# hustvl/LSFA

Hardware: AMD Instinct MI355X
Metric: frames/sec/GPU at 1000x600 key_interval=10 (whole-job frames/s) (higher is better)
Workload: dtype f32

## Files before the change

### lsfa_amd/csrc/conv_ring_kernel.h

```cpp
#pragma once
#include "conv_split_kernel.h"

namespace lsfa {
namespace convsplit {

constexpr int kFlush = 12;

#ifndef LSFA_RING_A_AUX
#define LSFA_RING_A_AUX 0
#endif
#ifndef LSFA_RING_B_AUX
#define LSFA_RING_B_AUX 0
#endif

#ifdef LSFA_LAB_HALF_A
constexpr int kRingIssueA = 2;
#else
constexpr int kRingIssueA = 4;
#endif

template <int NT, int PC, int ST, int WV = 4> struct Ring {
  static constexpr int kColTile = 128 * PC;
  static constexpr int kStageA = WV * 256;
  static constexpr int kStageBn = NT * kColTile;
  static constexpr int kStageN = kStageA + kStageBn;
  static constexpr int kDmaB = (NT * kColTile) / (WV * 64);
  static constexpr int kDma = kRingIssueA + kDmaB;
  static constexpr int kLdsBytes = ST * kStageN * 16;
  static constexpr int kWgPerCu = (2 * kLdsBytes <= 160 * 1024) ? 2 : 1;
  static_assert((NT * kColTile) % (WV * 64) == 0, "NT * PC must be a multiple of WV / 2");
  static_assert(kLdsBytes <= 160 * 1024, "ring does not fit the CU's LDS");
  static_assert((ST - 1) * kDma <= 63, "vmcnt is a 6-bit counter");
};

__device__ __forceinline__ float4 affine_relu4(const float4& v, const float4& sc, const float4& sh) {
  return make_float4(fmaxf(v.x * sc.x + sh.x, 0.f), fmaxf(v.y * sc.y + sh.y, 0.f), fmaxf(v.z * sc.z + sh.z, 0.f), fmaxf(v.w * sc.w + sh.w, 0.f));
}
__device__ __forceinline__ void affine_chunk(const float* T, int gch, int lane, float4& c0, float4& c1, float4& c2, float4& c3) {
  const float4* sc = reinterpret_cast<const float4*>(T + gch * kChunk + 16 * (lane >> 5));
  const float4* sh = reinterpret_cast<const float4*>(T + kAffineMaxCin + gch * kChunk + 16 * (lane >> 5));
  c0 = affine_relu4(c0, sc[0], sh[0]);
  c1 = affine_relu4(c1, sc[1], sh[1]);
  c2 = affine_relu4(c2, sc[2], sh[2]);
  c3 = affine_relu4(c3, sc[3], sh[3]);
}

template <int NT, int PC, int ST, int WV, int S>
__device__ __forceinline__ void ring_issue_a(uint4 (*R)[(Ring<NT, PC, ST, WV>::kStageN)], const float* __restrict__ x, const Geom& g, const Walk& wk, bool live) {
  const int dy = wk.ty * g.dil, dx = wk.tx * g.dil;
  const int doff = (dy * g.W + dx) * g.lda + wk.kc * kChunk;
  const int dy_b = live ? dy : (1 << 26);
  uint4* a_dst = &R[S][g.wave * 256];
#pragma unroll
  for (int i = 0; i < kRingIssueA; ++i) {
    const bool ok = (unsigned)(g.iy0[i] + dy_b) < (unsigned)g.H && (unsigned)(g.ix0[i] + dx) < (unsigned)g.W;
    const float* src = ok ? x + (g.off0[i] + doff) : g_zero_block;
    __builtin_amdgcn_global_load_lds(reinterpret_cast<const uint4*>(src), a_dst + i * 64, 16, 0, LSFA_RING_A_AUX);
  }
}

template <int NT, int PC, int ST, int WV, int S, int I0, int I1>
__device__ __forceinline__ void ring_issue_b(uint4 (*R)[(Ring<NT, PC, ST, WV>::kStageN)], const uint4* __restrict__ wblock, const Geom& g, int gch) {
  typedef Ring<NT, PC, ST, WV> RG;
  const uint4* wsrc = wblock + (size_t)gch * g.wstride + g.wave * (RG::kDmaB * 64) + g.lane;
  uint4* b_dst = &R[S][RG::kStageA + g.wave * (RG::kDmaB * 64)];
#pragma unroll
  for (int i = I0; i < I1; ++i) __builtin_amdgcn_global_load_lds(wsrc + i * 64, b_dst + i * 64, 16, 0, LSFA_RING_B_AUX);
}

template <int NT, int PC, int ST, int WV, int S, bool PIPE>
__device__ __forceinline__ void ring_issue_chunk(uint4 (*R)[(Ring<NT, PC, ST, WV>::kStageN)], const float* __restrict__ x, const uint4* __restrict__ wblock,
                                                 const Geom& g, Walk& wk, bool live) {
  ring_issue_a<NT, PC, ST, WV, S>(R, x, g, wk, PIPE ? live : true);
  ring_issue_b<NT, PC, ST, WV, S, 0, Ring<NT, PC, ST, WV>::kDmaB>(R, wblock, g, PIPE ? wk.bprev : wk.bidx);
  wk.next(g.kh, g.kw, g.chunks_per_tap, g.k_order);
}

template <int NT, int PC, int ST, int WV, int S, bool PIPE, bool GUARD>
__device__ __forceinline__ void ring_prologue(uint4 (*R)[(Ring<NT, PC, ST, WV>::kStageN)], const float* __restrict__ x, const uint4* __restrict__ wblock,
                                              const Geom& g, Walk& wk, int n) {
  if (!GUARD || S < n) ring_issue_chunk<NT, PC, ST, WV, S, PIPE>(R, x, wblock, g, wk, S + 1 < n);
}

template <int ST, int kDma>
__device__ __forceinline__ void wait_chunks_ahead(int ahead) {
  if (ST >= 4 && ahead >= 2) wait_vmcnt<(ST >= 4 ? 2 : 0) * kDma>();
  else if (ST >= 3 && ahead == 1) wait_vmcnt<(ST >= 3 ? 1 : 0) * kDma>();
  else wait_vmcnt<0>();
}

struct Cut { PiecesN s0, s1; };

template <int PC, bool AF>
__device__ __forceinline__ Cut cut_rows(const uint4& r0, const uint4& r1, const uint4& r2, const uint4& r3, float a_scale, const float* T, int gch, int lane) {
  float4 c0 = as_f4(r0), c1 = as_f4(r1), c2 = as_f4(r2), c3 = as_f4(r3);
  if (AF) affine_chunk(T, gch, lane, c0, c1, c2, c3);
  Cut n;
  n.s0 = cut8<PC>(c0, c1, AF ? 1.f : a_scale);
  n.s1 = cut8<PC>(c2, c3, AF ? 1.f : a_scale);
  return n;
}

template <int PC, bool AF> struct CutCost { static constexpr int kValu = (PC == 2 ? 64 : PC == 3 ? 96 : 16) + (AF ? 48 : 0); };

template <int NT, int PC, bool AF, int DMA = 0, int WV = 4> __device__ __forceinline__ void pin_interleave() {
  if (PC == 3 && NT == 4) return;
  constexpr int kMfma = NT * 2 * (PC == 3 ? 6 : PC == 2 ? 3 : 1);
  constexpr int kPer = (CutCost<PC, AF>::kValu + (DMA ? 24 : 0) + kMfma - 1) / kMfma + 1;
  __builtin_amdgcn_sched_group_barrier(0x100, ((PC == 3 || WV == 8) ? PC + 2 : 2 * PC + 4) + (AF ? 8 : 0), 0);
#pragma unroll
  for (int i = 0; i < kMfma; ++i) {
    __builtin_amdgcn_sched_group_barrier(0x008, 1, 0);
    __builtin_amdgcn_sched_group_barrier(0x100, 1, 0);
    if (i >= 1 && i <= DMA) __builtin_amdgcn_sched_group_barrier(0x010, 1, 0);
    __builtin_amdgcn_sched_group_barrier(0x002, kPer, 0);
  }
}

template <int NT, int PC, int ST, int WV, int S, bool AF, int DMA = 0>
__device__ __forceinline__ Cut ring_mma_cut(const uint4 (*R)[(Ring<NT, PC, ST, WV>::kStageN)], const Geom& g, const Cut& p, f32x16 (&acc)[NT], float a_scale,
                                            int gch_next, const float* T) {
  const uint4* B = &R[S][Ring<NT, PC, ST, WV>::kStageA + g.lane];
  const uint4* A = &R[S][g.wave * 256];
  uint4 bf[NT * 2][PC];
#pragma unroll
  for (int q = 0; q < PC; ++q) bf[0][q] = B[q * 64];
  const uint4 r0 = A[g.frag[0]], r1 = A[g.frag[1]];
#pragma unroll
  for (int t = 1; t < NT; ++t)
#pragma unroll
    for (int q = 0; q < PC; ++q) bf[t * 2][q] = B[((t * 2) * PC + q) * 64];
  const uint4 r2 = A[g.frag[2]], r3 = A[g.frag[3]];
#pragma unroll
  for (int t = 0; t < NT; ++t)
#pragma unroll
    for (int q = 0; q < PC; ++q) bf[t * 2 + 1][q] = B[((t * 2 + 1) * PC + q) * 64];
  const Cut n = cut_rows<PC, AF>(r0, r1, r2, r3, a_scale, T, min(gch_next, g.chunks_per_tap - 1), g.lane);
#pragma unroll
  for (int t = 0; t < NT; ++t) acc[t] = mma_pc<PC>(p.s0, bf[t * 2][0], bf[t * 2][PC > 1 ? 1 : 0], bf[t * 2][PC > 2 ? 2 : 0], acc[t]);
#pragma unroll
  for (int t = 0; t < NT; ++t) acc[t] = mma_pc<PC>(p.s1, bf[t * 2 + 1][0], bf[t * 2 + 1][PC > 1 ? 1 : 0], bf[t * 2 + 1][PC > 2 ? 2 : 0], acc[t]);
  pin_interleave<NT, PC, AF, DMA, WV>();
  return n;
}

template <int NT, int PC, int ST, int WV, int S, bool AF>
__device__ __forceinline__ Cut ring_cut(const uint4 (*R)[(Ring<NT, PC, ST, WV>::kStageN)], const Geom& g, float a_scale, int gch, const float* T) {
  const uint4* A = &R[S][g.wave * 256];
  const uint4 r0 = A[g.frag[0]], r1 = A[g.frag[1]], r2 = A[g.frag[2]], r3 = A[g.frag[3]];
  return cut_rows<PC, AF>(r0, r1, r2, r3, a_scale, T, min(gch, g.chunks_per_tap - 1), g.lane);
}

template <int NT, int PC, int ST, int WV, int S, bool AF>
__device__ __forceinline__ void ring_step_uniform(uint4 (*R)[(Ring<NT, PC, ST, WV>::kStageN)], const float* __restrict__ x, const uint4* __restrict__ wblock,
                                                  const Geom& g, Walk& wk, int v, int n, f32x16 (&acc)[NT], Cut& p, float a_scale, const float* T) {
  typedef Ring<NT, PC, ST, WV> RG;
  constexpr int SN = (S + ST - 1) % ST;
  wait_vmcnt<(ST - 2) * RG::kDma>();
  asm volatile("s_waitcnt lgkmcnt(0)" ::: "memory");
  __builtin_amdgcn_s_barrier();
  const Walk cur = wk;
  wk.next(g.kh, g.kw, g.chunks_per_tap, g.k_order);
  ring_issue_a<NT, PC, ST, WV, SN>(R, x, g, cur, v + ST < n);
  ring_issue_b<NT, PC, ST, WV, SN, 0, RG::kDmaB>(R, wblock, g, cur.bprev);
  p = ring_mma_cut<NT, PC, ST, WV, S, AF, RG::kDma>(R, g, p, acc, a_scale, g.chunk0 + v + 1, T);
}

template <int NT, int PC, int ST, int WV, int S, bool PIPE>
__device__ __forceinline__ void ring_load_step(uint4 (*R)[(Ring<NT, PC, ST, WV>::kStageN)], const float* __restrict__ x, const uint4* __restrict__ wblock,
                                               const Geom& g, Walk& wk, int v, int n) {
  typedef Ring<NT, PC, ST, WV> RG;
  constexpr int SN = (S + ST - 1) % ST;
  wait_chunks_ahead<ST, RG::kDma>(min(n - 1 - v, ST - 2));
  __builtin_amdgcn_s_barrier();
  if (v + ST - 1 < n) ring_issue_chunk<NT, PC, ST, WV, SN, PIPE>(R, x, wblock, g, wk, v + ST < n);
}

template <int NT, int PC, int ST, int WV, int S, bool AF>
__device__ __forceinline__ void ring_consume_step(uint4 (*R)[(Ring<NT, PC, ST, WV>::kStageN)], const Geom& g, f32x16 (&acc)[NT], Cut& p, float a_scale, int v,
                                                  const float* T) {
  asm volatile("s_waitcnt lgkmcnt(0)" ::: "memory");
  __builtin_amdgcn_s_barrier();
  p = ring_mma_cut<NT, PC, ST, WV, S, AF>(R, g, p, acc, a_scale, g.chunk0 + v + 1, T);
}

template <int NT, int PC, int ST, int WV>
__device__ __forceinline__ void ring_wait_first(int n) {
  typedef Ring<NT, PC, ST, WV> RG;
  const int behind = min(n, ST - 1);
  if (ST >= 4 && behind >= 3) wait_vmcnt<(ST >= 4 ? 3 : 0) * RG::kDma>();
  else if (ST >= 3 && behind == 2) wait_vmcnt<(ST >= 3 ? 2 : 0) * RG::kDma>();
  else if (behind == 1) wait_vmcnt<RG::kDma>();
  else wait_vmcnt<0>();
}

template <int NT, int PC, int ST, int S, bool AF, bool COPIES>
__device__ __forceinline__ void ring_step_r4(uint4 (*R)[(Ring<NT, PC, ST, 4>::kStageN)], const float* __restrict__ x, const uint4* __restrict__ wblock,
                                          const Geom& g, Walk& wk, int c, int n, f32x16 (&acc)[NT], float a_scale, const float* T) {
  typedef Ring<NT, PC, ST, 4> RG;
  constexpr int kDmaB = RG::kDmaB;
  constexpr int SN = (S + ST - 1) % ST;
  if (COPIES) wait_chunks_ahead<ST, RG::kDma>(min(n - 1 - c, ST - 2));
  asm volatile("s_waitcnt lgkmcnt(0)" ::: "memory");
  __builtin_amdgcn_s_barrier();
  const bool more = COPIES && c + ST - 1 < n;
  const int gch_next = wk.bidx;
  if (more) ring_issue_a<NT, PC, ST, 4, SN>(R, x, g, wk, true);
  const uint4* A = &R[S][g.wave * 256];
  const uint4* B = &R[S][Ring<NT, PC, ST, 4>::kStageA + g.lane];
  const uint4 r0 = A[g.frag[0]], r1 = A[g.frag[1]], r2 = A[g.frag[2]], r3 = A[g.frag[3]];
  float4 c0 = as_f4(r0), c1 = as_f4(r1), c2 = as_f4(r2), c3 = as_f4(r3);
  if (AF) affine_chunk(T, g.chunk0 + c, g.lane, c0, c1, c2, c3);
  const PiecesN s0 = cut8<PC>(c0, c1, AF ? 1.f : a_scale), s1 = cut8<PC>(c2, c3, AF ? 1.f : a_scale);
#pragma unroll
  for (int t = 0; t < NT; ++t) {
    acc[t] = mma_pc<PC>(s0, B + ((t * 2 + 0) * PC) * 64, acc[t]);
    acc[t] = mma_pc<PC>(s1, B + ((t * 2 + 1) * PC) * 64, acc[t]);
    if (more) {
      constexpr int kPer = (kDmaB + NT - 1) / NT;
      constexpr int kE0 = (kPer < kDmaB) ? kPer : kDmaB;
      constexpr int kE1 = (2 * kPer < kDmaB) ? 2 * kPer : kDmaB;
      constexpr int kE2 = (3 * kPer < kDmaB) ? 3 * kPer : kDmaB;
      if (t == 0) ring_issue_b<NT, PC, ST, 4, SN, 0, kE0>(R, wblock, g, gch_next);
      if (NT > 1 && t == 1) ring_issue_b<NT, PC, ST, 4, SN, kE0, (NT > 2 ? kE1 : kDmaB)>(R, wblock, g, gch_next);
      if (NT > 2 && t == 2) ring_issue_b<NT, PC, ST, 4, SN, kE1, (NT > 3 ? kE2 : kDmaB)>(R, wblock, g, gch_next);
      if (NT > 3 && t == 3) ring_issue_b<NT, PC, ST, 4, SN, kE2, kDmaB>(R, wblock, g, gch_next);
    }
  }
  if (more) wk.next(g.kh, g.kw, g.chunks_per_tap, g.k_order);
}

template <int NT, int PC, int ST, bool SP = false, bool AF = false, int WV = 4>
static __global__ __launch_bounds__((SP || WV == 8 ? 2 : 1) * kThreads,
    WV == 8 ? 2 : (((AF ? 2 * (Ring<NT, PC, ST, WV>::kLdsBytes + 16384) <= 160 * 1024 : Ring<NT, PC, ST, WV>::kWgPerCu == 2) && !(SP && NT == 4)) ? 2 : 1) * (SP ? 2 : 1))
void conv_ring_kernel(Args a, int nx, int ny, int nz) {
  typedef Ring<NT, PC, ST, WV> RG;
  __shared__ __attribute__((aligned(16))) uint4 R[ST][RG::kStageN];
  __shared__ __attribute__((aligned(16))) float T[AF ? 2 * kAffineMaxCin : 4];
  Tile tile = xcd_tile(blockIdx.x, nx, ny, nz, a.tile_order, a.inv_nx, a.inv_ny);
  if (tile.x < 0) return;
  if (a.nphase > 1) { const int slices = nz / a.nphase, phase = tile.z / slices; tile.z -= phase * slices; apply_phase(a, phase, slices); }
  const int tid = threadIdx.x;
  const int P = a.N * a.Ho * a.Wo;
  static_assert(!(SP && WV != 4), "loader / consumer waves exist for 128-pixel tiles only");
  constexpr int kPix = 32 * WV;
  constexpr bool kUniform = !SP && (WV == 8 || NT == 4);
  constexpr bool kPipelined = (SP && NT == 4) || kUniform;
  if (tile.x * kPix >= P) return;
  const int taps = a.kh * a.kw;
  Geom g;
  g.lane = tid & 63;
  const int wave8 = __builtin_amdgcn_readfirstlane(tid >> 6);
  const bool loader = SP && wave8 >= 4;
  g.wave = WV == 8 ? wave8 : (wave8 & 3);
  float a_scale = 1.f;
  float out_scale[NT];
#pragma unroll
  for (int t = 0; t < NT; ++t) out_scale[t] = 1.f;
  ScaleRegs sr;
  if (PC == 2 && !loader) scale_loads_issue<NT>(a, tile.y * (32 * NT), g.lane, sr);
#ifdef LSFA_LAB_EARLY_SCALES
  constexpr bool kScalesEarly = true;
#else
  constexpr bool kScalesEarly = false;
#endif
#define LSFA_SCALES_READY(N_)                                                                                                   \
  if (!kScalesEarly || (N_) < 0) {                                                                                              \
    if (PC == 2) { scale_loads_wait<((N_) < 0 ? 0 : (N_))>(sr); a_scale = scale_finish<NT>(a, sr, g.lane, out_scale); }         \
    if (AF) {                                                                                                                   \
      for (int k = tid; k < a.Cin; k += 64 * WV) { T[k] = a.in_scale[k] * a_scale; T[kAffineMaxCin + k] = a.in_shift[k] * a_scale; } \
    }                                                                                                                           \
  }
  if (kScalesEarly && !loader) LSFA_SCALES_READY(-1)
  g.H = a.H; g.W = a.W; g.Cin = a.Cin; g.lda = a.lda; g.kh = a.kh; g.kw = a.kw; g.stride = a.stride; g.dil = a.dil;
  g.k_order = taps > 1 ? a.k_order : 0;
  g.chunks_per_tap = a.Cin / kChunk;
  const int chunk_total = taps * g.chunks_per_tap;
  g.chunk0 = tile.z * a.chunks_per_slice;
  const int nchunks = min(a.chunks_per_slice, chunk_total - g.chunk0);
  const int col_tiles = a.Cout / 32;
  g.wstride = (size_t)col_tiles * RG::kColTile;
  const uint4* wblock = a.wfrag + (size_t)(NT * tile.y) * RG::kColTile;
  const int m0 = tile.x * kPix + g.wave * kWavePix;
  if (!SP || loader) {
#pragma unroll
  for (int i = 0; i < 4; ++i) {
    const int pix = m0 + 8 * i + (g.lane >> 3);
    const int piece = LSFA_DMA_SRC_PIECE(i, g.lane);
    g.iy0[i] = g.ix0[i] = -(1 << 24);
    g.off0[i] = 0;
    if (pix < P) {
      const int pn = fdiv(pix, a.Ho * a.Wo, a.inv_howo), r = pix - pn * a.Ho * a.Wo, py = fdiv(r, a.Wo, a.inv_wo), px = r - py * a.Wo;
      g.iy0[i] = py * a.stride - a.pad_h;
      g.ix0[i] = px * a.stride - a.pad_w;
      g.off0[i] = ((pn * a.H + g.iy0[i]) * a.W + g.ix0[i]) * a.lda + 4 * piece;
    }
  }
  }
  LSFA_FRAG_SLOTS(g.lane, g.frag)
  f32x16 acc[NT];
#pragma unroll
  for (int t = 0; t < NT; ++t)
#pragma unroll
    for (int i = 0; i < 16; ++i) acc[t][i] = 0.f;

  Walk wk;
  wk.start(g.chunk0, a.kh, a.kw, g.chunks_per_tap, g.k_order);
  f32x16 sum[NT];
#pragma unroll
  for (int t = 0; t < NT; ++t)
#pragma unroll
    for (int i = 0; i < 16; ++i) sum[t][i] = 0.f;
  if constexpr (!kPipelined) {
    if (SP) {
      if (loader) {
        ring_prologue<NT, PC, ST, 4, 0, false, true>(R, a.x, wblock, g, wk, nchunks);
        if (ST > 2) ring_prologue<NT, PC, ST, 4, (ST > 2 ? 1 : 0), false, true>(R, a.x, wblock, g, wk, nchunks);
        if (ST > 3) ring_prologue<NT, PC, ST, 4, (ST > 3 ? 2 : 0), false, true>(R, a.x, wblock, g, wk, nchunks);
        for (int c = 0; c < nchunks; c += ST) {
          ring_load_step<NT, PC, ST, 4, 0, false>(R, a.x, wblock, g, wk, c, nchunks);
          if (c + 1 < nchunks) ring_load_step<NT, PC, ST, 4, 1, false>(R, a.x, wblock, g, wk, c + 1, nchunks);
          if (ST > 2 && c + 2 < nchunks) ring_load_step<NT, PC, ST, 4, (ST > 2 ? 2 : 0), false>(R, a.x, wblock, g, wk, c + 2, nchunks);
          if (ST > 3 && c + 3 < nchunks) ring_load_step<NT, PC, ST, 4, (ST > 3 ? 3 : 0), false>(R, a.x, wblock, g, wk, c + 3, nchunks);
        }
        return;
      }
      LSFA_SCALES_READY(0)
      int since = 0;
      for (int c = 0; c < nchunks; c += ST) {
        ring_step_r4<NT, PC, ST, 0, AF, false>(R, a.x, wblock, g, wk, c, nchunks, acc, a_scale, T);
        if (c + 1 < nchunks) ring_step_r4<NT, PC, ST, 1, AF, false>(R, a.x, wblock, g, wk, c + 1, nchunks, acc, a_scale, T);
        if (ST > 2 && c + 2 < nchunks) ring_step_r4<NT, PC, ST, (ST > 2 ? 2 : 0), AF, false>(R, a.x, wblock, g, wk, c + 2, nchunks, acc, a_scale, T);
        if (ST > 3 && c + 3 < nchunks) ring_step_r4<NT, PC, ST, (ST > 3 ? 3 : 0), AF, false>(R, a.x, wblock, g, wk, c + 3, nchunks, acc, a_scale, T);
        since += ST;
        if (since >= kFlush) {
          since = 0;
  #pragma unroll
          for (int t = 0; t < NT; ++t)
  #pragma unroll
            for (int i = 0; i < 16; ++i) { sum[t][i] = sum[t][i] + acc[t][i]; acc[t][i] = 0.f; }
        }
      }
    } else {
      ring_prologue<NT, PC, ST, 4, 0, false, true>(R, a.x, wblock, g, wk, nchunks);
      if (ST > 2) ring_prologue<NT, PC, ST, 4, (ST > 2 ? 1 : 0), false, true>(R, a.x, wblock, g, wk, nchunks);
      if (ST > 3) ring_prologue<NT, PC, ST, 4, (ST > 3 ? 2 : 0), false, true>(R, a.x, wblock, g, wk, nchunks);
      LSFA_SCALES_READY(0)
      int since = 0;
      for (int c = 0; c < nchunks; c += ST) {
        ring_step_r4<NT, PC, ST, 0, AF, true>(R, a.x, wblock, g, wk, c, nchunks, acc, a_scale, T);
        if (c + 1 < nchunks) ring_step_r4<NT, PC, ST, 1, AF, true>(R, a.x, wblock, g, wk, c + 1, nchunks, acc, a_scale, T);
        if (ST > 2 && c + 2 < nchunks) ring_step_r4<NT, PC, ST, (ST > 2 ? 2 : 0), AF, true>(R, a.x, wblock, g, wk, c + 2, nchunks, acc, a_scale, T);
        if (ST > 3 && c + 3 < nchunks) ring_step_r4<NT, PC, ST, (ST > 3 ? 3 : 0), AF, true>(R, a.x, wblock, g, wk, c + 3, nchunks, acc, a_scale, T);
        since += ST;
        if (since >= kFlush) {
          since = 0;
  #pragma unroll
          for (int t = 0; t < NT; ++t)
  #pragma unroll
            for (int i = 0; i < 16; ++i) { sum[t][i] = sum[t][i] + acc[t][i]; acc[t][i] = 0.f; }
        }
      }
    }
  } else {
  if (SP && loader) {
    ring_issue_a<NT, PC, ST, WV, ST - 1>(R, a.x, g, wk, true);
    wk.next(g.kh, g.kw, g.chunks_per_tap, g.k_order);
    ring_prologue<NT, PC, ST, WV, 0, true, true>(R, a.x, wblock, g, wk, nchunks);
    if (ST > 2) ring_prologue<NT, PC, ST, WV, (ST > 2 ? 1 : 0), true, true>(R, a.x, wblock, g, wk, nchunks);
    if (ST > 3) ring_prologue<NT, PC, ST, WV, (ST > 3 ? 2 : 0), true, true>(R, a.x, wblock, g, wk, nchunks);
    ring_wait_first<NT, PC, ST, WV>(nchunks);
    __builtin_amdgcn_s_barrier();
    for (int c = 0; c < nchunks; c += ST) {
      ring_load_step<NT, PC, ST, WV, 0, true>(R, a.x, wblock, g, wk, c, nchunks);
      if (c + 1 < nchunks) ring_load_step<NT, PC, ST, WV, 1, true>(R, a.x, wblock, g, wk, c + 1, nchunks);
      if (ST > 2 && c + 2 < nchunks) ring_load_step<NT, PC, ST, WV, (ST > 2 ? 2 : 0), true>(R, a.x, wblock, g, wk, c + 2, nchunks);
      if (ST > 3 && c + 3 < nchunks) ring_load_step<NT, PC, ST, WV, (ST > 3 ? 3 : 0), true>(R, a.x, wblock, g, wk, c + 3, nchunks);
    }
    return;
  }
  if (kUniform) {
    ring_issue_a<NT, PC, ST, WV, ST - 1>(R, a.x, g, wk, true);
    wk.next(g.kh, g.kw, g.chunks_per_tap, g.k_order);
    ring_prologue<NT, PC, ST, WV, 0, true, false>(R, a.x, wblock, g, wk, nchunks);
    if (ST > 2) ring_prologue<NT, PC, ST, WV, (ST > 2 ? 1 : 0), true, false>(R, a.x, wblock, g, wk, nchunks);
    if (ST > 3) ring_prologue<NT, PC, ST, WV, (ST > 3 ? 2 : 0), true, false>(R, a.x, wblock, g, wk, nchunks);
    wait_vmcnt<(ST - 1) * RG::kDma>();
    LSFA_SCALES_READY((ST - 1) * RG::kDma)
  } else {
    LSFA_SCALES_READY(0)
  }
  asm volatile("s_waitcnt lgkmcnt(0)" ::: "memory");
  __builtin_amdgcn_s_barrier();
  Cut p = ring_cut<NT, PC, ST, WV, ST - 1, AF>(R, g, a_scale, g.chunk0, T);
  {
    int since = 0;
    for (int c = 0; c < nchunks; c += ST) {
      if (SP) {
        ring_consume_step<NT, PC, ST, WV, 0, AF>(R, g, acc, p, a_scale, c, T);
        if (c + 1 < nchunks) ring_consume_step<NT, PC, ST, WV, 1, AF>(R, g, acc, p, a_scale, c + 1, T);
        if (ST > 2 && c + 2 < nchunks) ring_consume_step<NT, PC, ST, WV, (ST > 2 ? 2 : 0), AF>(R, g, acc, p, a_scale, c + 2, T);
        if (ST > 3 && c + 3 < nchunks) ring_consume_step<NT, PC, ST, WV, (ST > 3 ? 3 : 0), AF>(R, g, acc, p, a_scale, c + 3, T);
      } else if (kUniform) {
        ring_step_uniform<NT, PC, ST, WV, 0, AF>(R, a.x, wblock, g, wk, c, nchunks, acc, p, a_scale, T);
        if (c + 1 < nchunks) ring_step_uniform<NT, PC, ST, WV, 1, AF>(R, a.x, wblock, g, wk, c + 1, nchunks, acc, p, a_scale, T);
        if (ST > 2 && c + 2 < nchunks) ring_step_uniform<NT, PC, ST, WV, (ST > 2 ? 2 : 0), AF>(R, a.x, wblock, g, wk, c + 2, nchunks, acc, p, a_scale, T);
        if (ST > 3 && c + 3 < nchunks) ring_step_uniform<NT, PC, ST, WV, (ST > 3 ? 3 : 0), AF>(R, a.x, wblock, g, wk, c + 3, nchunks, acc, p, a_scale, T);
      }
      since += ST;
      if (since >= kFlush) {
        since = 0;
#pragma unroll
        for (int t = 0; t < NT; ++t)
#pragma unroll
          for (int i = 0; i < 16; ++i) { sum[t][i] = sum[t][i] + acc[t][i]; acc[t][i] = 0.f; }
      }
    }
  }
  }
#pragma unroll
  for (int t = 0; t < NT; ++t)
#pragma unroll
    for (int i = 0; i < 16; ++i) acc[t][i] = (sum[t][i] + acc[t][i]) * out_scale[t];

  const int lane = g.lane;
  if (kUniform) wait_vmcnt<0>();
  constexpr bool kRowsFit = RG::kLdsBytes >= WV * NT * 4096;
  const bool rows_ok = kRowsFit && rows_path_ok(a);
  if (rows_ok) {
    float* part = a.part ? a.part + (size_t)tile.z * P * a.Cout : nullptr;
    RowsIn<NT> in;
    tile_rows_in<NT>(a, m0, P, tile.y * (32 * NT), part != nullptr, lane, in);
    asm volatile("s_waitcnt lgkmcnt(0)" ::: "memory");
    __builtin_amdgcn_s_barrier();
    float* T = reinterpret_cast<float*>(&R[0][0]) + g.wave * (NT * 1024);
#pragma unroll
    for (int t = 0; t < NT; ++t)
#pragma unroll
      for (int r = 0; r < 16; ++r) T[t * 1024 + acc_row(r, lane) * 32 + (lane & 31)] = acc[t][r];
    const uint32_t m = tile_rows_out<NT>(a, T, m0, P, tile.y * (32 * NT), part, lane, in);
    if (!part) publish_amax(m, a.amax_out, a.status, blockIdx.x * WV + g.wave);
    return;
  }
  constexpr bool kColsFit = RG::kLdsBytes >= WV * NT * 32 * kColPitch * 4;
  if (kColsFit && a.y_nchw && !a.part && !a.view) {
    asm volatile("s_waitcnt lgkmcnt(0)" ::: "memory");
    __builtin_amdgcn_s_barrier();
    float* Tc = reinterpret_cast<float*>(&R[0][0]) + g.wave * (NT * 32 * kColPitch);
#pragma unroll
    for (int t = 0; t < NT; ++t)
#pragma unroll
      for (int r = 0; r < 16; ++r) Tc[acc_row(r, lane, (t * 32 + (lane & 31)) * kColPitch)] = acc[t][r];
    asm volatile("s_waitcnt lgkmcnt(0)" ::: "memory");
    const uint32_t m = tile_cols_out_nchw<NT>(a, Tc, m0, P, tile.y * (32 * NT), lane);
    publish_amax(m, a.amax_out, a.status, blockIdx.x * WV + g.wave);
    return;
  }
  int prow[16];
  RowOut ro;
  ro.valid = 0;
#pragma unroll
  for (int r = 0; r < 16; ++r) {
    prow[r] = acc_row(r, lane, m0);
    if (prow[r] < P) ro.valid |= 1u << r;
  }
  if (a.part) {
    float* part = a.part + (size_t)tile.z * P * a.Cout;
#pragma unroll
    for (int t = 0; t < NT; ++t) tile_store_part(part, a.Cout, prow, ro.valid, tile.y * (32 * NT) + t * 32 + (lane & 31), acc[t]);
    return;
  }
#pragma unroll
  for (int r = 0; r < 16; ++r) ro.base[r] = ((ro.valid >> r) & 1u) ? out_pixel_base(a, prow[r]) : 0;
  uint32_t m = 0;
#pragma unroll
  for (int t = 0; t < NT; ++t) m = max(m, tile_store_max(a, ro, tile.y * (32 * NT) + t * 32 + (lane & 31), acc[t]));
  publish_amax(m, a.amax_out, a.status, blockIdx.x * WV + g.wave);
}

#undef LSFA_SCALES_READY

template <int PC>
static __global__ void pack_weights_kernel(const float* __restrict__ w, uint4* __restrict__ out, int Cout, int taps, int Cin, int w_exp,
                                           const int* __restrict__ w_exp_pc = nullptr) {
  const int col_tiles = Cout / 32, chunks = Cin / kChunk;
  const long total = (long)taps * chunks * col_tiles * 2 * 64;
  const long i = (long)blockIdx.x * blockDim.x + threadIdx.x;
  if (i >= total) return;
  const int lane = (int)(i & 63);
  long r = i >> 6;
  const int s = (int)(r & 1); r >>= 1;
  const int t = (int)(r % col_tiles); r /= col_tiles;
  const int g = (int)r;
  const int tap = g / chunks, kc = g - tap * chunks;
  const int co = t * 32 + (lane & 31);
  const int ci = kc * kChunk + 16 * (lane >> 5) + 8 * s;
  const float* src = w + ((size_t)co * taps + tap) * Cin + ci;
  const float4 v0 = *reinterpret_cast<const float4*>(src), v1 = *reinterpret_cast<const float4*>(src + 4);
  const PiecesN p = cut8<PC>(v0, v1, ldexpf(1.f, w_exp_pc ? w_exp_pc[co] : w_exp));
  uint4* dst = out + ((((size_t)g * col_tiles + t) * 2 + s) * PC) * 64 + lane;
#pragma unroll
  for (int q = 0; q < PC; ++q) dst[q * 64] = p.p[q];
}

}
}
```

Before: 3909.

## Add a third A-operand stage to the two-stage conv ring for one config

For the NT=4, PC=2, ST=2 uniform non-affine configuration, the LDS ring gains an extra activation (A) stage. A tiles are now prefetched three chunks ahead while weight (B) tiles stay double-buffered. The main loop is unrolled by six so the B stage (mod 2) and A stage (mod 3) indices stay compile-time constants, and the prologue and waitcnt values are adjusted to match. This aims to hide activation gather latency behind more MFMA work, at the cost of extra LDS that must still leave room for two workgroups per CU.

```diff
diff --git a/lsfa_amd/csrc/conv_ring_kernel.h b/lsfa_amd/csrc/conv_ring_kernel.h
--- a/lsfa_amd/csrc/conv_ring_kernel.h
+++ b/lsfa_amd/csrc/conv_ring_kernel.h
@@ -19,18 +19,37 @@
 constexpr int kRingIssueA = 4;
 #endif
 
-template <int NT, int PC, int ST, int WV = 4> struct Ring {
+#ifndef LSFA_RING_DEEP_A
+#define LSFA_RING_DEEP_A 1
+#endif
+template <int NT, int PC, int ST, bool SP, bool AF, int WV> constexpr int ring_depth_a() {
+  return (LSFA_RING_DEEP_A && NT == 4 && PC == 2 && ST == 2 && !SP && !AF && WV == 4) ? ST + 1 : ST;
+}
+
+template <int NT, int PC, int ST, int WV = 4, int DA = ST> struct Ring {
   static constexpr int kColTile = 128 * PC;
   static constexpr int kStageA = WV * 256;
   static constexpr int kStageBn = NT * kColTile;
   static constexpr int kStageN = kStageA + kStageBn;
   static constexpr int kDmaB = (NT * kColTile) / (WV * 64);
   static constexpr int kDma = kRingIssueA + kDmaB;
-  static constexpr int kLdsBytes = ST * kStageN * 16;
+  static constexpr int kStages = ST, kDepthA = DA;
+  static constexpr int kLdsN = ST * kStageN + (DA - ST) * kStageA;
+  static constexpr int kLdsBytes = kLdsN * 16;
   static constexpr int kWgPerCu = (2 * kLdsBytes <= 160 * 1024) ? 2 : 1;
   static_assert((NT * kColTile) % (WV * 64) == 0, "NT * PC must be a multiple of WV / 2");
   static_assert(kLdsBytes <= 160 * 1024, "ring does not fit the CU's LDS");
-  static_assert((ST - 1) * kDma <= 63, "vmcnt is a 6-bit counter");
+  static_assert((ST - 1) * kDma + (DA - ST) * kRingIssueA <= 63, "vmcnt is a 6-bit counter");
+  static_assert(DA == ST || DA == ST + 1, "at most one A stage beyond the [A | B] stages");
+};
+
+template <class RG, bool DEEP = (RG::kDepthA > RG::kStages)> struct RingImage {
+  typedef uint4 type[RG::kStages][RG::kStageN];
+  __device__ static __forceinline__ type& stages(type& img) { return img; }
+};
+template <class RG> struct RingImage<RG, true> {
+  struct type { uint4 s[RG::kStages][RG::kStageN]; uint4 a[(RG::kDepthA - RG::kStages) * RG::kStageA]; };
+  __device__ static __forceinline__ uint4 (&stages(type& img))[RG::kStages][RG::kStageN] { return img.s; }
 };
 
 __device__ __forceinline__ float4 affine_relu4(const float4& v, const float4& sc, const float4& sh) {
@@ -117,11 +136,11 @@
   }
 }
 
-template <int NT, int PC, int ST, int WV, int S, bool AF, int DMA = 0>
+template <int NT, int PC, int ST, int WV, int S, bool AF, int DMA = 0, int SA = S>
 __device__ __forceinline__ Cut ring_mma_cut(const uint4 (*R)[(Ring<NT, PC, ST, WV>::kStageN)], const Geom& g, const Cut& p, f32x16 (&acc)[NT], float a_scale,
                                             int gch_next, const float* T) {
   const uint4* B = &R[S][Ring<NT, PC, ST, WV>::kStageA + g.lane];
-  const uint4* A = &R[S][g.wave * 256];
+  const uint4* A = &R[SA][g.wave * 256];
   uint4 bf[NT * 2][PC];
 #pragma unroll
   for (int q = 0; q < PC; ++q) bf[0][q] = B[q * 64];
@@ -164,6 +183,24 @@
   ring_issue_a<NT, PC, ST, WV, SN>(R, x, g, cur, v + ST < n);
   ring_issue_b<NT, PC, ST, WV, SN, 0, RG::kDmaB>(R, wblock, g, cur.bprev);
   p = ring_mma_cut<NT, PC, ST, WV, S, AF, RG::kDma>(R, g, p, acc, a_scale, g.chunk0 + v + 1, T);
+}
+
+template <int NT, int PC, int ST, int WV, int V6, bool AF>
+__device__ __forceinline__ void ring_step_deep_a(uint4 (*R)[(Ring<NT, PC, ST, WV>::kStageN)], const float* __restrict__ x, const uint4* __restrict__ wblock,
+                                                 const Geom& g, Walk& wk, int& bq, int v, int n, f32x16 (&acc)[NT], Cut& p, float a_scale, const float* T) {
+  typedef Ring<NT, PC, ST, WV, ST + 1> RG;
+  static_assert(ST == 2, "B stage v % 2, A stage k % 3");
+  constexpr int SB = V6 % 2, SBN = (V6 + 1) % 2;
+  constexpr int SA = (V6 + 1) % 3, SAN = V6 % 3;
+  wait_vmcnt<kRingIssueA>();
+  asm volatile("s_waitcnt lgkmcnt(0)" ::: "memory");
+  __builtin_amdgcn_s_barrier();
+  const Walk cur = wk;
+  wk.next(g.kh, g.kw, g.chunks_per_tap, g.k_order);
+  ring_issue_b<NT, PC, ST, WV, SBN, 0, RG::kDmaB>(R, wblock, g, bq);
+  ring_issue_a<NT, PC, ST, WV, SAN>(R, x, g, cur, v + 3 < n);
+  bq = cur.bprev;
+  p = ring_mma_cut<NT, PC, ST, WV, SB, AF, RG::kDma, SA>(R, g, p, acc, a_scale, g.chunk0 + v + 1, T);
 }
 
 template <int NT, int PC, int ST, int WV, int S, bool PIPE>
@@ -232,11 +269,15 @@
 
 template <int NT, int PC, int ST, bool SP = false, bool AF = false, int WV = 4>
 static __global__ __launch_bounds__((SP || WV == 8 ? 2 : 1) * kThreads,
-    WV == 8 ? 2 : (((AF ? 2 * (Ring<NT, PC, ST, WV>::kLdsBytes + 16384) <= 160 * 1024 : Ring<NT, PC, ST, WV>::kWgPerCu == 2) && !(SP && NT == 4)) ? 2 : 1) * (SP ? 2 : 1))
+    WV == 8 ? 2 : (((AF ? 2 * (Ring<NT, PC, ST, WV>::kLdsBytes + 16384) <= 160 * 1024 : Ring<NT, PC, ST, WV, ring_depth_a<NT, PC, ST, SP, AF, WV>()>::kWgPerCu == 2) && !(SP && NT == 4)) ? 2 : 1) * (SP ? 2 : 1))
 void conv_ring_kernel(Args a, int nx, int ny, int nz) {
-  typedef Ring<NT, PC, ST, WV> RG;
-  __shared__ __attribute__((aligned(16))) uint4 R[ST][RG::kStageN];
+  constexpr bool kDeepA = ring_depth_a<NT, PC, ST, SP, AF, WV>() > ST;
+  typedef Ring<NT, PC, ST, WV, ring_depth_a<NT, PC, ST, SP, AF, WV>()> RG;
+  __shared__ __attribute__((aligned(16))) typename RingImage<RG>::type Rimg;
+  uint4 (&R)[ST][RG::kStageN] = RingImage<RG>::stages(Rimg);
   __shared__ __attribute__((aligned(16))) float T[AF ? 2 * kAffineMaxCin : 4];
+  static_assert(sizeof(Rimg) == RG::kLdsBytes, "the ring's image is what Ring says it is");
+  static_assert(!kDeepA || (RG::kWgPerCu == 2 && !AF), "the third A stage must not cost the second workgroup of a CU");
   Tile tile = xcd_tile(blockIdx.x, nx, ny, nz, a.tile_order, a.inv_nx, a.inv_ny);
   if (tile.x < 0) return;
   if (a.nphase > 1) { const int slices = nz / a.nphase, phase = tile.z / slices; tile.z -= phase * slices; apply_phase(a, phase, slices); }
@@ -379,7 +420,20 @@
     }
     return;
   }
-  if (kUniform) {
+  int bq = 0;
+  if constexpr (kDeepA) {
+    const int b0 = wk.bidx;
+    ring_issue_a<NT, PC, ST, WV, 0>(R, a.x, g, wk, true);
+    wk.next(g.kh, g.kw, g.chunks_per_tap, g.k_order);
+    bq = wk.bidx;
+    ring_issue_a<NT, PC, ST, WV, 1>(R, a.x, g, wk, 1 < nchunks);
+    wk.next(g.kh, g.kw, g.chunks_per_tap, g.k_order);
+    ring_issue_b<NT, PC, ST, WV, 0, 0, RG::kDmaB>(R, wblock, g, b0);
+    ring_issue_a<NT, PC, ST, WV, 2>(R, a.x, g, wk, 2 < nchunks);
+    wk.next(g.kh, g.kw, g.chunks_per_tap, g.k_order);
+    wait_vmcnt<RG::kDma + kRingIssueA>();
+    LSFA_SCALES_READY(RG::kDma + kRingIssueA)
+  } else if (kUniform) {
     ring_issue_a<NT, PC, ST, WV, ST - 1>(R, a.x, g, wk, true);
     wk.next(g.kh, g.kw, g.chunks_per_tap, g.k_order);
     ring_prologue<NT, PC, ST, WV, 0, true, false>(R, a.x, wblock, g, wk, nchunks);
@@ -392,8 +446,27 @@
   }
   asm volatile("s_waitcnt lgkmcnt(0)" ::: "memory");
   __builtin_amdgcn_s_barrier();
-  Cut p = ring_cut<NT, PC, ST, WV, ST - 1, AF>(R, g, a_scale, g.chunk0, T);
-  {
+  Cut p = ring_cut<NT, PC, ST, WV, kDeepA ? 0 : ST - 1, AF>(R, g, a_scale, g.chunk0, T);
+  if constexpr (kDeepA) {
+    static_assert(kFlush % 6 == 0, "the flush points must not depend on the ring");
+    int since = 0;
+    for (int c = 0; c < nchunks; c += 6) {
+      ring_step_deep_a<NT, PC, ST, WV, 0, AF>(R, a.x, wblock, g, wk, bq, c, nchunks, acc, p, a_scale, T);
+      if (c + 1 < nchunks) ring_step_deep_a<NT, PC, ST, WV, 1, AF>(R, a.x, wblock, g, wk, bq, c + 1, nchunks, acc, p, a_scale, T);
+      if (c + 2 < nchunks) ring_step_deep_a<NT, PC, ST, WV, 2, AF>(R, a.x, wblock, g, wk, bq, c + 2, nchunks, acc, p, a_scale, T);
+      if (c + 3 < nchunks) ring_step_deep_a<NT, PC, ST, WV, 3, AF>(R, a.x, wblock, g, wk, bq, c + 3, nchunks, acc, p, a_scale, T);
+      if (c + 4 < nchunks) ring_step_deep_a<NT, PC, ST, WV, 4, AF>(R, a.x, wblock, g, wk, bq, c + 4, nchunks, acc, p, a_scale, T);
+      if (c + 5 < nchunks) ring_step_deep_a<NT, PC, ST, WV, 5, AF>(R, a.x, wblock, g, wk, bq, c + 5, nchunks, acc, p, a_scale, T);
+      since += 6;
+      if (since >= kFlush) {
+        since = 0;
+#pragma unroll
+        for (int t = 0; t < NT; ++t)
+#pragma unroll
+          for (int i = 0; i < 16; ++i) { sum[t][i] = sum[t][i] + acc[t][i]; acc[t][i] = 0.f; }
+      }
+    }
+  } else {
     int since = 0;
     for (int c = 0; c < nchunks; c += ST) {
       if (SP) {
@@ -425,7 +498,7 @@
 
   const int lane = g.lane;
   if (kUniform) wait_vmcnt<0>();
-  constexpr bool kRowsFit = RG::kLdsBytes >= WV * NT * 4096;
+  constexpr bool kRowsFit = Ring<NT, PC, ST, WV>::kLdsBytes >= WV * NT * 4096;
   const bool rows_ok = kRowsFit && rows_path_ok(a);
   if (rows_ok) {
     float* part = a.part ? a.part + (size_t)tile.z * P * a.Cout : nullptr;
@@ -442,7 +515,7 @@
     if (!part) publish_amax(m, a.amax_out, a.status, blockIdx.x * WV + g.wave);
     return;
   }
-  constexpr bool kColsFit = RG::kLdsBytes >= WV * NT * 32 * kColPitch * 4;
+  constexpr bool kColsFit = Ring<NT, PC, ST, WV>::kLdsBytes >= WV * NT * 32 * kColPitch * 4;
   if (kColsFit && a.y_nchw && !a.part && !a.view) {
     asm volatile("s_waitcnt lgkmcnt(0)" ::: "memory");
     __builtin_amdgcn_s_barrier();
```

After: 3965 (median of 6 runs). 1.4% higher.
